# kkromberg/SpeechRecognition

Hardware: AMD Instinct MI355X
Metric: frames/sec scored+decoded (higher is better)
Workload: dtype f64

## Files before the change

### speechrecognition_amd/csrc/gmm_prefilter.hip

```cpp
#include <hip/hip_runtime.h>
#include <stdint.h>

#include <algorithm>
#include <cmath>
#include <vector>

#include "kernels.h"

#ifndef SR_P16_NB
#define SR_P16_NB 4
#endif

namespace srgpu {

typedef float v4f __attribute__((ext_vector_type(4)));
static constexpr int kPWaves = 4;
static constexpr int kGroupBlocks = 8;

typedef _Float16 f16x8 __attribute__((ext_vector_type(8)));

__device__ inline uint32_t pack_f16x2(_Float16 l, _Float16 h) {
  return (uint32_t)__builtin_bit_cast(uint16_t, l) | ((uint32_t)__builtin_bit_cast(uint16_t, h) << 16);
}

// ... 330 lines not shown
  if (e == hipSuccess) e = hipStreamSynchronize(stream);
  if (e == hipSuccess) e = hipMemcpy(h, d, sizeof(h), hipMemcpyDeviceToHost);
  (void)hipFree(d);
  if (e != hipSuccess) return e;
  *preserved = true;
  for (int i = 0; i < 64; i++) *preserved = *preserved && h[i] == 9.765625e-4f;
  return hipSuccess;
}

template <int KS>
__global__ void fp16_accumulation_probe_kernel(const _Float16* A, const _Float16* B, float* out) {
  constexpr int K = 32 * KS;
  const int lane = threadIdx.x, r = lane & 15, q = lane >> 4;
  v4f acc = {0.f, 0.f, 0.f, 0.f};
#pragma unroll
  for (int ks = 0; ks < KS; ks++) {
    f16x8 a, b;
#pragma unroll
    for (int j = 0; j < 8; j++) {
      const int k = 32 * ks + 8 * q + j;
      a[j] = A[r * K + k];
      b[j] = B[k * 16 + r];
    }
    acc = __builtin_amdgcn_mfma_f32_16x16x32_f16(a, b, acc, 0, 0, 0);
  }
#pragma unroll
  for (int i = 0; i < 4; i++) out[(4 * q + i) * 16 + r] = acc[i];
}

hipError_t probe_fp16_accumulation(hipStream_t stream, int ks32, bool* ok, double* worst_ratio) {
  if (ks32 != 3 && ks32 != 4) return hipErrorInvalidValue;
  const int kCases = 8;
  const int K = 32 * ks32;
  const double allowed = ks32 == 3 ? 87.0 : 132.0;
  std::vector<_Float16> hA((size_t)kCases * 16 * K), hB((size_t)kCases * K * 16);
  uint64_t rng = 0x9E3779B97F4A7C15ull;
  auto next = [&]() { rng ^= rng << 13; rng ^= rng >> 7; rng ^= rng << 17; return rng; };
  for (int t = 0; t < kCases; t++) {
    _Float16* A = hA.data() + (size_t)t * 16 * K;
    _Float16* B = hB.data() + (size_t)t * K * 16;
    for (int k = 0; k < K; k++)
      for (int c = 0; c < 16; c++) B[k * 16 + c] = (_Float16)1.0f;
    for (int r = 0; r < 16; r++)
      for (int k = 0; k < K; k++) {
        float a = 0.f;
        const int fam = (t * 16 + r) & 3;
        if (fam == 0) a = k == (r * 5) % K ? 4096.0f : 0.75f;
        else if (fam == 1) a = k >= K - 2 ? 0.f : ((k & 1) ? -1.f : 1.f) * (1024.0f + (float)(((k >> 1) * 7 + r) % 64) * ((k & 1) ? 0.5f : 0.53125f));
        else if (fam == 2) a = 1.0009765625f;
        else { const uint64_t u = next(); a = ((u & 1) ? -1.f : 1.f) * (1.0f + (float)((u >> 8) & 1023) / 1024.0f) * (float)(1u << ((u >> 20) % 12)); }
        A[r * K + k] = (_Float16)a;
      }
    for (int k = 0; k < K; k++)
      for (int c = 0; c < 16; c++) {
        const uint64_t u = next();
        float b = 1.0f + (float)((u >> 5) % 1024) / 1024.0f;
        if ((c & 3) == 0) b = 1.0f;
        if ((c & 3) == 1) b = 1.0009765625f;
        B[k * 16 + c] = (_Float16)b;
      }
    for (int c = 0; c < 16; c++)
      for (int r = 0; r < 16; r++)
        if (((t * 16 + r) & 3) == 0) B[((r * 5) % K) * 16 + c] = (_Float16)2048.0f;
  }
  _Float16 *dA = nullptr, *dB = nullptr;
  float* dO = nullptr;
  hipError_t e;
  if ((e = hipMalloc(reinterpret_cast<void**>(&dA), hA.size() * 2)) != hipSuccess) return e;
  if ((e = hipMalloc(reinterpret_cast<void**>(&dB), hB.size() * 2)) != hipSuccess) { (void)hipFree(dA); return e; }
  if ((e = hipMalloc(reinterpret_cast<void**>(&dO), (size_t)kCases * 256 * 4)) != hipSuccess) { (void)hipFree(dA); (void)hipFree(dB); return e; }
  std::vector<float> got((size_t)kCases * 256);
  e = hipMemcpy(dA, hA.data(), hA.size() * 2, hipMemcpyHostToDevice);
  if (e == hipSuccess) e = hipMemcpy(dB, hB.data(), hB.size() * 2, hipMemcpyHostToDevice);
  for (int t = 0; t < kCases && e == hipSuccess; t++) {
    if (ks32 == 3) hipLaunchKernelGGL(fp16_accumulation_probe_kernel<3>, dim3(1), dim3(64), 0, stream, dA + (size_t)t * 16 * K, dB + (size_t)t * K * 16, dO + (size_t)t * 256);
    else hipLaunchKernelGGL(fp16_accumulation_probe_kernel<4>, dim3(1), dim3(64), 0, stream, dA + (size_t)t * 16 * K, dB + (size_t)t * K * 16, dO + (size_t)t * 256);
    e = hipGetLastError();
  }
  if (e == hipSuccess) e = hipStreamSynchronize(stream);
  if (e == hipSuccess) e = hipMemcpy(got.data(), dO, got.size() * 4, hipMemcpyDeviceToHost);
  (void)hipFree(dA); (void)hipFree(dB); (void)hipFree(dO);
  if (e != hipSuccess) return e;
  double worst = 0.0;
  bool fine = true;
  for (int t = 0; t < kCases; t++)
    for (int r = 0; r < 16; r++)
      for (int c = 0; c < 16; c++) {
        double exact = 0.0, mag = 0.0;
        for (int k = 0; k < K; k++) {
          const double p = (double)(float)hA[((size_t)t * 16 + r) * K + k] * (double)(float)hB[((size_t)t * K + k) * 16 + c];
          exact += p;
          mag += p < 0 ? -p : p;
        }
        const double err = std::fabs((double)got[(size_t)t * 256 + r * 16 + c] - exact);
        const double ratio = err / (mag * 5.9604644775390625e-8);
        if (!(ratio <= allowed)) fine = false;
        if (ratio > worst || ratio != ratio) worst = ratio;
      }
  *ok = fine;
  if (worst_ratio) *worst_ratio = worst;
  return hipSuccess;
}

static GmmStationaryPlan stationary_plan(uint32_t n_groups, uint64_t n_frames) {
  GmmStationaryPlan p{};
  p.n_quads = (n_groups + kPWaves - 1) / kPWaves;
  const uint64_t steps = (n_frames + 16 * kSNB - 1) / (16 * kSNB);
  const uint64_t r_max = std::max<uint64_t>(1, std::min<uint64_t>(steps, (n_frames + kSRangeFrames - 1) / kSRangeFrames));
  uint64_t best_r = 1;
  double best = -1.0;
  for (uint64_t r = 1; r <= r_max; r++) {
    const uint64_t wgs = (uint64_t)p.n_quads * r;
    const double fill = (double)wgs / (double)((wgs + 511) / 512 * 512);
    if (fill > best * (1.0 + 1e-9)) { best = fill; best_r = r; }
  }
  const uint64_t range_steps = (steps + best_r - 1) / best_r;
  p.range_frames = (uint32_t)(range_steps * 16 * kSNB);
  p.n_ranges = (uint32_t)((steps + range_steps - 1) / range_steps);
  p.per_xcd = (uint32_t)(((uint64_t)p.n_quads * p.n_ranges + 7) / 8);
  return p;
}

int gmm_prefilter_route(int ks32, int route) { return (route == kPfStationary && ks32 >= 1 && ks32 <= 3) ? kPfStationary : kPfStaged; }
int gmm_prefilter_stationary_range_frames() { return kSRangeFrames; }
void gmm_prefilter_operand_sizes(int ks32, uint64_t n_frames, size_t* n_frag, size_t* n_norm) {
  const uint64_t blocks = (n_frames + 16 * kSNB - 1) / (16 * kSNB) * kSNB;
  *n_frag = (size_t)blocks * ks32 * 64;
  *n_norm = (size_t)blocks * 16;
}

template <int KS32>
static hipError_t launch_stationary(const GmmPrefilterArgs& a, hipStream_t stream) {
  if (!a.bfrag || !a.bnorm || a.n_groups == 0) return hipErrorInvalidValue;
  size_t n_frag, n_norm;
  gmm_prefilter_operand_sizes(KS32, a.n_frames, &n_frag, &n_norm);
  const uint64_t blocks = n_norm / 16;
  hipLaunchKernelGGL((gmm_prefilter_operands_kernel<KS32>), dim3((unsigned)((blocks + kPWaves - 1) / kPWaves)), dim3(kPWaves * 64), 0, stream,
                     a.feats, a.n_frames, a.dim, blocks, a.bfrag, a.bnorm);
  hipError_t e = hipGetLastError();
  if (e != hipSuccess) return e;
  const GmmStationaryPlan p = stationary_plan(a.n_groups, a.n_frames);
  hipLaunchKernelGGL((gmm_prefilter_stationary_kernel<KS32>), dim3(8 * p.per_xcd), dim3(kPWaves * 64), 0, stream, a, p);
  return hipGetLastError();
}

hipError_t launch_gmm_prefilter(const GmmPrefilterArgs& a, int ks32, int route, hipStream_t stream) {
  if (a.n_frames >= (1ull << 30)) return hipErrorInvalidValue;
  if (a.n_frames == 0) return hipSuccess;
  if (gmm_prefilter_route(ks32, route) == kPfStationary) {
    switch (ks32) {
      case 1: return launch_stationary<1>(a, stream);
      case 2: return launch_stationary<2>(a, stream);
      default: return launch_stationary<3>(a, stream);
    }
  }
  const dim3 grid(a.nx * a.ny), block(kPWaves * 64);
  switch (ks32) {
    case 1: hipLaunchKernelGGL((gmm_prefilter16_kernel<1, SR_P16_NB>), grid, block, 0, stream, a); break;
    case 2: hipLaunchKernelGGL((gmm_prefilter16_kernel<2, SR_P16_NB>), grid, block, 0, stream, a); break;
    case 3: hipLaunchKernelGGL((gmm_prefilter16_kernel<3, SR_P16_NB>), grid, block, 0, stream, a); break;
    case 4: hipLaunchKernelGGL((gmm_prefilter16_kernel<4, SR_P16_NB>), grid, block, 0, stream, a); break;
    default: return hipErrorInvalidValue;
  }
  return hipGetLastError();
}
int gmm_prefilter_frames_per_tile() { return kPWaves * SR_P16_NB * 16; }

#pragma clang fp contract(off)

#ifndef SR_R_THREADS
#define SR_R_THREADS 768
#endif
#ifndef SR_R_BATCH
#define SR_R_BATCH 4
#endif
static constexpr int kRThreads = SR_R_THREADS;
static constexpr int kRThreadsWide = 512;
static constexpr int kRWaves = kRThreads / 64;
static constexpr int kRBatch = SR_R_BATCH;
#ifndef SR_R_BATCH_WIDE
#define SR_R_BATCH_WIDE 8
#endif
static constexpr int kRBatchWide = SR_R_BATCH_WIDE;
static constexpr uint32_t kRingEntries = 128;
static constexpr uint32_t kRingLists = 2 * 8 * kRingEntries;
static constexpr uint32_t kRingWave = 4 * kRingLists;
struct __attribute__((aligned(16))) RingEntry { uint32_t lf, mask; double score; };
struct __attribute__((packed, aligned(4))) RowPiece { float v[4]; };

template <int DT, int NS, int SPW, int CH, int NT = kRThreads, int VS = 1, bool DEFER = false>
__global__ __launch_bounds__(NT) void gmm_refine_kernel(GmmRefineArgs a) {
  static_assert(DT > 0 && (DT & 1), "padded dimension: odd");
  static_assert(!DEFER || CH > 1, "deferred lists: states of several chunks");
  constexpr int kRThreads = NT, kRWaves = NT / 64;
  static_assert(CH == 1 || CH == 2 || CH == 4, "chunks per state (half)");
  static_assert(VS == 1 || (VS == 2 && CH == 4), "two halves only of four-chunk states");
  static_assert(SPW % (CH * VS) == 0 && (CH == 1 || SPW % 4 == 0), "a state's chunks live in one workgroup");
  extern __shared__ __attribute__((aligned(1024))) unsigned char panel_raw[];
  const uint32_t D = (uint32_t)DT, tid = threadIdx.x;
  const int lane = tid & 63, wave = tid >> 6;
  const uint32_t s0 = blockIdx.x * SPW;
  const uint32_t ns = (s0 + SPW <= a.n_pstates) ? SPW : a.n_pstates - s0;
  const uint32_t state_bytes = (2u * D + 2u) * NS * 8u;
  const uint64_t f_begin = (uint64_t)blockIdx.y * a.frames_per_split;
  const uint64_t f_end = (f_begin + a.frames_per_split < a.n_frames) ? f_begin + a.frames_per_split : a.n_frames;

  {
    const uint32_t chunks = (ns * state_bytes + 1023u) >> 10;
    const unsigned char* src = reinterpret_cast<const unsigned char*>(a.rows) + (uint64_t)s0 * state_bytes + lane * 16;
    for (uint32_t ch = wave; ch < chunks; ch += kRWaves)
      __builtin_amdgcn_global_load_lds((const __attribute__((address_space(1))) void*)(src + (uint64_t)ch * 1024u),
                                       (__attribute__((address_space(3))) void*)(panel_raw + ch * 1024u), 16, 0, 0);
  }
  uint32_t nd[SPW];
#pragma unroll
  for (int j = 0; j < SPW; j++) nd[j] = (uint32_t)j < ns ? a.n_dens_ps[s0 + j] : 0u;
  __builtin_amdgcn_s_waitcnt(0x0F70);
  __syncthreads();
  if (f_begin >= f_end) return;

  uint32_t n_eval = 0;
  double x[DT];
  const __amdgpu_buffer_rsrc_t featsT_rsrc = __builtin_amdgcn_make_buffer_rsrc(
      const_cast<float*>(a.featsT), 0, (int)0xFFFFFFFFu, 0x00020000);
  const uint32_t ld4 = (uint32_t)a.n_frames_ld * 4u;
  auto load_x = [&](uint64_t f) __attribute__((always_inline)) {
    const uint32_t voff = (uint32_t)f * 4u;
#pragma unroll
    for (int k = 0; k < DT; k++)
      x[k] = (double)__builtin_bit_cast(float, __builtin_amdgcn_raw_buffer_load_b32(featsT_rsrc, voff, (uint32_t)k * ld4, 0));
  };
  auto load_x_row = [&](uint64_t f) __attribute__((always_inline)) {
    const float* xr = a.feats + f * (uint64_t)DT;
#pragma unroll
    for (int q = 0; q < DT / 4; q++) {
      const RowPiece t = reinterpret_cast<const RowPiece*>(xr)[q];
#pragma unroll
      for (int i = 0; i < 4; i++) x[4 * q + i] = (double)t.v[i];
    }
#pragma unroll
    for (int k = DT - DT % 4; k < DT; k++) x[k] = (double)xr[k];
  };
  auto evaluate = [&](const unsigned char* col0) __attribute__((always_inline)) -> double {
    const volatile __attribute__((address_space(3))) double* col =
        (const volatile __attribute__((address_space(3))) double*)col0;
    double l0 = 0.0, l1 = 0.0, dist, score;
    {
      constexpr int RB = NT == kRThreadsWide ? kRBatchWide : kRBatch;
      constexpr int NB_ = (DT + 1 + RB - 1) / RB;
      double pm[2][RB], pv[2][RB];
#pragma unroll
      for (int i = 0; i < RB; i++)
        if (i <= DT) { pm[0][i] = col[(2 * i) * NS]; pv[0][i] = col[(2 * i + 1) * NS]; }
#pragma unroll
      for (int b = 0; b < NB_; b++) {
        const int cur = b & 1;
        __builtin_amdgcn_sched_barrier(0);
#pragma unroll
        for (int i = 0; i < RB; i++) {
          const int k = (b + 1) * RB + i;
          if (k <= DT) { pm[cur ^ 1][i] = col[(2 * k) * NS]; pv[cur ^ 1][i] = col[(2 * k + 1) * NS]; }
        }
        __builtin_amdgcn_sched_barrier(0);
#pragma unroll
        for (int i = 0; i < RB; i++) {
          const int k = b * RB + i;
          if (k < (int)(DT - (DT & 1))) {
            double u = x[k] - pm[cur][i];
            u = u * u;
            u = u * pv[cur][i];
            if (k & 1) l1 = l1 + u; else l0 = l0 + u;
          } else if (k == DT - 1) {
            dist = l0 + l1;
            const double t = x[k] - pm[cur][i];
            dist += t * t * pv[cur][i];
          } else if (k == DT) {
            if (!(DT & 1)) dist = l0 + l1;
            score = pm[cur][i] + dist / 2;
            score -= pv[cur][i];
          }
        }
        asm volatile("" : "+v"(l0), "+v"(l1));
      }
    }
    return score;
  };

  const double seed = 1e10;
  auto seeded_min = [&](double score) -> double {
    double r;
    asm("v_min_f64 %0, %1, %2" : "=v"(r) : "v"(score), "s"(seed));
    return r;
  };
  RingEntry* ring = reinterpret_cast<RingEntry*>(a.ring + ((uint64_t)(blockIdx.y * gridDim.x + blockIdx.x) * kRWaves + wave) * kRingWave);
  const bool counting = a.n_refined != nullptr;
  uint64_t cnt1 = 0, cnt2 = 0;
  const uint64_t wave_global = (uint64_t)(blockIdx.y * gridDim.x + blockIdx.x) * kRWaves + wave;
  RingEntry* seg = DEFER ? reinterpret_cast<RingEntry*>(a.defer) + wave_global * SPW * (uint64_t)a.defer_cap : nullptr;
  uint32_t dcnt[DEFER ? SPW : 1];
  if constexpr (DEFER) {
#pragma unroll
    for (int j = 0; j < SPW; j++) dcnt[j] = 0;
  }
  const uint64_t f_wave = f_begin + (uint64_t)wave * 64;
  auto frame_of = [&](uint32_t lf) -> uint64_t { return f_wave + (uint64_t)(lf >> 6) * kRThreads + (lf & 63u); };
  const uint32_t chunk_shift = CH == 1 ? (a.chunks == 1 ? 0u : a.chunks == 2 ? 1u : 2u) : CH == 2 ? 1u : VS == 2 ? 3u : 2u;

  const uint32_t n_it = (uint32_t)((f_end - f_begin + kRThreads - 1) / kRThreads);
  for (uint32_t it = 0; it < n_it; it++) {
    const uint64_t fr = f_wave + (uint64_t)it * kRThreads + lane;
    const bool valid = fr < f_end;
    const uint64_t f = valid ? fr : f_end - 1;
    const uint32_t lf = it * 64u + (uint32_t)lane;
    load_x(f);
    constexpr int RS = SPW / (CH * VS);
    double res[RS];
    if constexpr (CH == 1) {
#pragma unroll
      for (int h = 0; h < SPW / 4; h++) {
        const uint4 v = reinterpret_cast<const uint4*>(a.mask)[(uint64_t)((s0 >> 2) + h) * a.n_frames + f];
        const uint32_t mk[4] = {v.x, v.y, v.z, v.w};
#pragma unroll
        for (int jj = 0; jj < 4; jj++) {
          const int j = 4 * h + jj;
          const uint32_t n = nd[j];
          uint32_t mask = mk[jj];
          mask &= n >= 32 ? 0xFFFFFFFFu : ((1u << n) - 1u);
          res[j] = 1e10;
          if (n) {
            const double score = evaluate(panel_raw + (size_t)j * state_bytes + (uint32_t)__builtin_ctz(mask | 0x80000000u) * 8u);
            res[j] = mask != 0 ? seeded_min(score) : res[j];
            if (counting) n_eval += (uint32_t)__builtin_popcountll(__ballot(valid));
          }
          const bool more = valid && (mask & (mask - 1)) != 0;
          const uint64_t b = __ballot(more);
          if (b) {
            const uint32_t c1 = (uint32_t)(cnt1 >> (8 * j)) & 0xFFu;
            const uint32_t pos = c1 + __builtin_amdgcn_mbcnt_hi((uint32_t)(b >> 32), __builtin_amdgcn_mbcnt_lo((uint32_t)b, 0u));
            if (more) {
              ring[(uint32_t)j * kRingEntries + pos] = RingEntry{lf, mask & (mask - 1), res[j]};
            }
            cnt1 += (uint64_t)__builtin_popcountll(b) << (8 * j);
          }
        }
      }
      if (valid) {
        if (a.chunks == 1) {
          double* o = a.out + f * a.ld + s0;
          if (ns == SPW) {
#pragma unroll
            for (int j = 0; j < SPW; j += 2) *reinterpret_cast<double2*>(o + j) = make_double2(res[j], res[j + 1]);
          } else {
#pragma unroll
            for (int j = 0; j < SPW; j++)
              if ((uint32_t)j < ns) o[j] = res[j];
          }
        } else if (a.chunks == 2) {
          double* o = a.out + f * a.ld + s0 / 2;
#pragma unroll
          for (int j = 0; j < SPW; j += 2) {
            const double m = res[j + 1] < res[j] ? res[j + 1] : res[j];
            if ((uint32_t)j < ns) o[j / 2] = m;
          }
        } else {
          double* o = a.out + f * a.ld + s0 / 4;
#pragma unroll
          for (int j = 0; j < SPW; j += 4) {
            double m = res[j + 1] < res[j] ? res[j + 1] : res[j];
            m = res[j + 2] < m ? res[j + 2] : m;
            m = res[j + 3] < m ? res[j + 3] : m;
            if ((uint32_t)j < ns) o[j / 4] = m;
          }
        }
      }
    } else {
      auto append = [&](int j, bool more, uint32_t rest, double& best) __attribute__((always_inline)) {
        const uint64_t b = __ballot(more);
        if (b) {
          if constexpr (DEFER) {
            const uint32_t nb = (uint32_t)__builtin_popcountll(b);
            if (dcnt[DEFER ? j : 0] + nb <= a.defer_cap) {
              const uint32_t pos = dcnt[DEFER ? j : 0] + __builtin_amdgcn_mbcnt_hi((uint32_t)(b >> 32), __builtin_amdgcn_mbcnt_lo((uint32_t)b, 0u));
              if (more) seg[(uint64_t)j * a.defer_cap + pos] = RingEntry{(uint32_t)f, rest, best};
              dcnt[DEFER ? j : 0] += nb;
            } else {
              uint32_t mm = more ? rest : 0u;
              const unsigned char* panel = panel_raw + (size_t)j * state_bytes;
              do {
                const double score = evaluate(panel + (uint32_t)__builtin_ctz(mm | 0x80000000u) * 8u);
                if (counting) n_eval += (uint32_t)__builtin_popcountll(__ballot(mm != 0));
                if (mm != 0 && score < best) best = score;
                mm &= mm - 1;
              } while (__any(mm != 0));
            }
          } else {
          const uint32_t c1 = (uint32_t)(cnt1 >> (8 * j)) & 0xFFu;
          const uint32_t pos = c1 + __builtin_amdgcn_mbcnt_hi((uint32_t)(b >> 32), __builtin_amdgcn_mbcnt_lo((uint32_t)b, 0u));
          if (more) {
            ring[(uint32_t)j * kRingEntries + pos] = RingEntry{lf, rest, best};
          }
          cnt1 += (uint64_t)__builtin_popcountll(b) << (8 * j);
          }
        }
      };
      uint32_t mk[SPW];
#pragma unroll
      for (int h = 0; h < SPW / 4; h++) {
        const uint4 v = reinterpret_cast<const uint4*>(a.mask)[(uint64_t)((s0 >> 2) + h) * a.n_frames + f];
        mk[4 * h] = v.x; mk[4 * h + 1] = v.y; mk[4 * h + 2] = v.z; mk[4 * h + 3] = v.w;
      }
#pragma unroll
      for (int j = 0; j < SPW; j++) mk[j] &= nd[j] >= 32 ? 0xFFFFFFFFu : ((1u << nd[j]) - 1u);
      if constexpr (VS == 1) {
#pragma unroll
      for (int r = 0; r < RS; r++) {
        uint32_t msel = mk[r * CH], off = 0;
#pragma unroll
        for (int c = 1; c < CH; c++) {
          const bool empty = msel == 0;
          msel = empty ? mk[r * CH + c] : msel;
          off = empty ? (uint32_t)c * state_bytes : off;
        }
        res[r] = 1e10;
        if (nd[r * CH]) {
          const double score = evaluate(panel_raw + (size_t)(r * CH) * state_bytes + off + (uint32_t)__builtin_ctz(msel | 0x80000000u) * 8u);
          res[r] = msel != 0 ? seeded_min(score) : res[r];
          if (counting) n_eval += (uint32_t)__builtin_popcountll(__ballot(valid));
        }
#pragma unroll
        for (int c = 0; c < CH; c++) {
          const bool is_sel = off == (uint32_t)c * state_bytes;
          const uint32_t rest = is_sel ? msel & (msel - 1) : mk[r * CH + c];
          if (nd[r * CH + c]) append(r * CH + c, valid && rest != 0, rest, res[r]);
        }
      }
      } else {
#pragma unroll
      for (int r = 0; r < RS; r++) res[r] = 1e10;
#pragma unroll
      for (int rv = 0; rv < RS * VS; rv++) {
        uint32_t msel = mk[rv * CH], off = 0;
#pragma unroll
        for (int c = 1; c < CH; c++) {
          const bool empty = msel == 0;
          msel = empty ? mk[rv * CH + c] : msel;
          off = empty ? (uint32_t)c * state_bytes : off;
        }
        double resv = 1e10;
        if (nd[rv * CH]) {
          const double score = evaluate(panel_raw + (size_t)(rv * CH) * state_bytes + off + (uint32_t)__builtin_ctz(msel | 0x80000000u) * 8u);
          resv = msel != 0 ? seeded_min(score) : resv;
          if (counting) n_eval += (uint32_t)__builtin_popcountll(__ballot(valid));
        }
        if constexpr (VS == 1) res[rv] = resv;
        else res[rv / VS] = resv < res[rv / VS] ? resv : res[rv / VS];
#pragma unroll
        for (int c = 0; c < CH; c++) {
          const bool is_sel = off == (uint32_t)c * state_bytes;
          const uint32_t rest = is_sel ? msel & (msel - 1) : mk[rv * CH + c];
          if (nd[rv * CH + c]) append(rv * CH + c, valid && rest != 0, rest, resv);
        }
        if constexpr (DEFER && VS == 2) res[rv / VS] = resv < res[rv / VS] ? resv : res[rv / VS];
      }
      }
      if (valid) {
        double* o = a.out + f * a.ld + s0 / (CH * VS);
        if (ns == SPW && RS >= 2) {
#pragma unroll
          for (int r = 0; r + 1 < RS; r += 2) *reinterpret_cast<double2*>(o + r) = make_double2(res[r], res[r + 1]);
        } else {
#pragma unroll
          for (int r = 0; r < RS; r++)
            if ((uint32_t)(r * CH * VS) < ns) o[r] = res[r];
        }
      }
    }
    const bool last = it + 1 == n_it;
    if constexpr (!DEFER)
    for (;;) {
      uint32_t level, j, n;
      {
        const uint64_t full1 = cnt1 & 0x4040404040404040ull, full2 = cnt2 & 0x4040404040404040ull;
        const uint64_t pick2 = full2 ? full2 : (last && !full1 && !cnt1) ? cnt2 : 0;
        const uint64_t pick1 = full2 ? 0 : full1 ? full1 : last ? cnt1 : 0;
        const uint64_t pick = pick1 ? pick1 : pick2;
        if (!pick) break;
        level = pick1 ? 1u : 2u;
        j = (uint32_t)__builtin_ctzll(pick) >> 3;
        const uint32_t have_ = (uint32_t)((pick1 ? cnt1 : cnt2) >> (8u * j)) & 0xFFu;
        n = have_ < 64u ? have_ : 64u;
      }
      asm volatile("" : "+s"(level), "+s"(j), "+s"(n));
      const bool l1 = level == 1;
      const uint32_t have = (uint32_t)((l1 ? cnt1 : cnt2) >> (8u * j)) & 0xFFu;
      const uint32_t slot0 = ((level - 1u) * 8u + j) * kRingEntries;
      if (l1) cnt1 -= (uint64_t)n << (8u * j); else cnt2 -= (uint64_t)n << (8u * j);
      const bool live = (uint32_t)lane < n;
      asm volatile("" ::: "memory");
      __builtin_amdgcn_fence(__ATOMIC_RELEASE, "wavefront");
      __builtin_amdgcn_fence(__ATOMIC_ACQUIRE, "wavefront");
      asm volatile("" ::: "memory");
      const uint32_t at = slot0 + have - n + (live ? (uint32_t)lane : 0u);
      const RingEntry en = ring[at];
      const uint32_t lfb = en.lf;
      uint32_t m = live ? en.mask : 0u;
      double cur = en.score;
      const uint64_t fb = frame_of(lfb);
      load_x_row(fb);
      double* o = a.out + fb * a.ld + ((s0 + j) >> chunk_shift);
      if constexpr (CH == 1) {
        if (chunk_shift) cur = *o;
      }
      const double before = cur;
      const unsigned char* panel = panel_raw + (size_t)j * state_bytes;
      do {
        const double score = evaluate(panel + (uint32_t)__builtin_ctz(m | 0x80000000u) * 8u);
        if (counting) n_eval += (uint32_t)__builtin_popcountll(__ballot(m != 0));
        if (m != 0 && score < cur) cur = score;
        m &= m - 1;
      } while (!l1 && __any(m != 0));
      if (l1) {
        const uint64_t b = __ballot(m != 0);
        if (b) {
          const uint32_t c2 = (uint32_t)(cnt2 >> (8u * j)) & 0xFFu;
          const uint32_t pos = c2 + __builtin_amdgcn_mbcnt_hi((uint32_t)(b >> 32), __builtin_amdgcn_mbcnt_lo((uint32_t)b, 0u));
          if (m != 0) {
            ring[(8u + j) * kRingEntries + pos] = RingEntry{lfb, m, cur};
          }
          cnt2 += (uint64_t)__builtin_popcountll(b) << (8u * j);
        }
      }
      asm volatile("" ::: "memory");
      const bool lower = live && cur < before;
      if constexpr (CH == 1) {
        if (lower) *o = cur;
      } else {
        __builtin_amdgcn_fence(__ATOMIC_RELEASE, "wavefront");
        if (lower) (void)__builtin_amdgcn_global_atomic_fmin_f64((__attribute__((address_space(1))) double*)o, cur);
      }
    }
  }
  if constexpr (DEFER) {
#pragma unroll
    for (int j = 0; j < SPW; j++)
      if (lane == 0) a.defer_cnt[wave_global * SPW + j] = dcnt[j];
  }
  if (a.n_refined) {
    if (lane == 0) atomicAdd(a.n_refined, (unsigned long long)n_eval);
  }
}

template <int DT, int NS, int SPW, int CH, int NT, int VS>
__global__ __launch_bounds__(NT) void gmm_drain_kernel(GmmRefineArgs a) {
  constexpr int kRWaves = NT / 64;
  constexpr int RB = kRBatch;
  extern __shared__ __attribute__((aligned(1024))) unsigned char panel_raw[];
  const uint32_t tid = threadIdx.x;
  const int lane = tid & 63, wave = tid >> 6;
  const uint32_t s0 = blockIdx.x * SPW;
  const uint32_t ns = (s0 + SPW <= a.n_pstates) ? SPW : a.n_pstates - s0;
  const uint32_t state_bytes = (2u * DT + 2u) * NS * 8u;
  {
    const uint32_t chunks = (ns * state_bytes + 1023u) >> 10;
    const unsigned char* src = reinterpret_cast<const unsigned char*>(a.rows) + (uint64_t)s0 * state_bytes + lane * 16;
    for (uint32_t ch = wave; ch < chunks; ch += kRWaves)
      __builtin_amdgcn_global_load_lds((const __attribute__((address_space(1))) void*)(src + (uint64_t)ch * 1024u),
                                       (__attribute__((address_space(3))) void*)(panel_raw + ch * 1024u), 16, 0, 0);
  }
  const uint64_t wave_global = (uint64_t)(blockIdx.y * gridDim.x + blockIdx.x) * kRWaves + wave;
  const RingEntry* seg = reinterpret_cast<const RingEntry*>(a.defer) + wave_global * SPW * (uint64_t)a.defer_cap;
  RingEntry* ring = reinterpret_cast<RingEntry*>(a.ring + wave_global * kRingWave) + 8u * kRingEntries;
  uint32_t nj[SPW];
#pragma unroll
  for (int j = 0; j < SPW; j++) nj[j] = (uint32_t)j < ns ? (uint32_t)__builtin_amdgcn_readfirstlane((int)a.defer_cnt[wave_global * SPW + j]) : 0u;
  __builtin_amdgcn_s_waitcnt(0x0F70);
  __syncthreads();
  const bool counting = a.n_refined != nullptr;
  uint32_t n_eval = 0;
  constexpr uint32_t chunk_shift = CH == 2 ? 1u : VS == 2 ? 3u : 2u;
  uint64_t cnt2 = 0;

  float xf[DT];
  auto load_row = [&](uint64_t f) __attribute__((always_inline)) {
    const float* xr = a.feats + f * (uint64_t)DT;
#pragma unroll
    for (int q = 0; q < DT / 4; q++) {
      const RowPiece t = reinterpret_cast<const RowPiece*>(xr)[q];
#pragma unroll
      for (int i = 0; i < 4; i++) xf[4 * q + i] = t.v[i];
    }
#pragma unroll
    for (int k = DT - DT % 4; k < DT; k++) xf[k] = xr[k];
  };
  auto evaluate = [&](const unsigned char* col0) __attribute__((always_inline)) -> double {
    const volatile __attribute__((address_space(3))) double* col = (const volatile __attribute__((address_space(3))) double*)col0;
    double l0 = 0.0, l1 = 0.0, dist, score;
    constexpr int NB_ = (DT + 1 + RB - 1) / RB;
    double pm[2][RB], pv[2][RB];
#pragma unroll
    for (int i = 0; i < RB; i++)
      if (i <= DT) { pm[0][i] = col[(2 * i) * NS]; pv[0][i] = col[(2 * i + 1) * NS]; }
#pragma unroll
    for (int b = 0; b < NB_; b++) {
      const int cur = b & 1;
      __builtin_amdgcn_sched_barrier(0);
#pragma unroll
      for (int i = 0; i < RB; i++) {
        const int k = (b + 1) * RB + i;
        if (k <= DT) { pm[cur ^ 1][i] = col[(2 * k) * NS]; pv[cur ^ 1][i] = col[(2 * k + 1) * NS]; }
      }
      __builtin_amdgcn_sched_barrier(0);
#pragma unroll
      for (int i = 0; i < RB; i++) {
        const int k = b * RB + i;
        if (k < DT - 1) {
          double u = (double)xf[k < DT ? k : 0] - pm[cur][i];
          u = u * u;
          u = u * pv[cur][i];
          if (k & 1) l1 = l1 + u; else l0 = l0 + u;
        } else if (k == DT - 1) {
          dist = l0 + l1;
          const double t = (double)xf[k < DT ? k : 0] - pm[cur][i];
          dist += t * t * pv[cur][i];
        } else if (k == DT) {
          score = pm[cur][i] + dist / 2;
          score -= pv[cur][i];
        }
      }
      asm volatile("" : "+v"(l0), "+v"(l1));
    }
    return score;
  };
  auto batch = [&](const bool l1, const uint32_t j, const RingEntry en, const bool live) __attribute__((always_inline)) {
    uint32_t m = live ? en.mask : 0u;
    double cur = en.score;
    const uint64_t fb = en.lf;
    load_row(fb);
    double* o = a.out + fb * a.ld + ((s0 + j) >> chunk_shift);
    const double before = cur;
    const unsigned char* panel = panel_raw + (size_t)j * state_bytes;
    do {
      const double score = evaluate(panel + (uint32_t)__builtin_ctz(m | 0x80000000u) * 8u);
      if (counting) n_eval += (uint32_t)__builtin_popcountll(__ballot(m != 0));
      if (m != 0 && score < cur) cur = score;
      m &= m - 1;
    } while (!l1 && __any(m != 0));
    if (l1) {
      const uint64_t b = __ballot(m != 0);
      if (b) {
        const uint32_t c2 = (uint32_t)(cnt2 >> (8u * j)) & 0xFFu;
        const uint32_t pos = c2 + __builtin_amdgcn_mbcnt_hi((uint32_t)(b >> 32), __builtin_amdgcn_mbcnt_lo((uint32_t)b, 0u));
        if (m != 0) ring[j * kRingEntries + pos] = RingEntry{en.lf, m, cur};
        cnt2 += (uint64_t)__builtin_popcountll(b) << (8u * j);
      }
    }
    if (live && cur < before) (void)__builtin_amdgcn_global_atomic_fmin_f64((__attribute__((address_space(1))) double*)o, cur);
  };
  auto level2 = [&](const bool flush) __attribute__((always_inline)) {
    for (;;) {
      const uint64_t pick = (cnt2 & 0x4040404040404040ull) ? (cnt2 & 0x4040404040404040ull) : flush ? cnt2 : 0ull;
      if (!pick) break;
      uint32_t j = (uint32_t)__builtin_ctzll(pick) >> 3;
      asm volatile("" : "+s"(j));
      const uint32_t have = (uint32_t)(cnt2 >> (8u * j)) & 0xFFu, n = have < 64u ? have : 64u;
      cnt2 -= (uint64_t)n << (8u * j);
      const bool live = (uint32_t)lane < n;
      asm volatile("" ::: "memory");
      __builtin_amdgcn_fence(__ATOMIC_RELEASE, "wavefront");
      __builtin_amdgcn_fence(__ATOMIC_ACQUIRE, "wavefront");
      asm volatile("" ::: "memory");
      const RingEntry en = ring[j * kRingEntries + have - n + (live ? (uint32_t)lane : 0u)];
      batch(false, j, en, live);
    }
  };
#pragma unroll 1
  for (uint32_t j = 0; j < ns; j++) {
    uint32_t n_left = 0;
#pragma unroll
    for (int q = 0; q < SPW; q++) n_left = (uint32_t)q == j ? nj[q] : n_left;
    const RingEntry* sj = seg + (uint64_t)j * a.defer_cap;
    RingEntry nxt = n_left ? sj[(uint32_t)lane < n_left ? lane : 0] : RingEntry{0u, 0u, 0.0};
#pragma unroll 1
    for (uint32_t pos = 0; pos < n_left; pos += 64u) {
      const RingEntry en = nxt;
      const uint32_t n = n_left - pos < 64u ? n_left - pos : 64u;
      const uint32_t p2 = pos + 64u;
      if (p2 < n_left) nxt = sj[p2 + ((uint32_t)lane < n_left - p2 ? lane : 0)];
      batch(true, j, en, (uint32_t)lane < n);
      level2(false);
    }
  }
  level2(true);
  if (a.n_refined) {
    if (lane == 0) atomicAdd(a.n_refined, (unsigned long long)n_eval);
  }
}

__device__ inline uint32_t padded_source_dim(uint32_t k, uint32_t dim, uint32_t dp) {
  const uint32_t pairs = dim - (dim & 1u);
  return k < pairs ? k : (k == dp - 1u && (dim & 1u)) ? dim - 1u : dim;
}
__global__ void transpose_feats_kernel(const float* feats, uint64_t n_frames, uint32_t dim, uint32_t dp, uint64_t ldT, float* out, float* featsP) {
  __shared__ float tile[64][65];
  const uint64_t f0 = (uint64_t)blockIdx.x * 64;
  for (uint32_t d0 = 0; d0 < dp; d0 += 64) {
    for (uint32_t i = threadIdx.x; i < 64 * 64; i += blockDim.x) {
      const uint32_t fr = i / 64, d = i % 64;
      const uint32_t src = d0 + d < dp ? padded_source_dim(d0 + d, dim, dp) : dim;
      tile[fr][d] = (f0 + fr < n_frames && src < dim) ? feats[(f0 + fr) * dim + src] : 0.0f;
    }
    __syncthreads();
    for (uint32_t i = threadIdx.x; i < 64 * 64; i += blockDim.x) {
      const uint32_t d = i / 64, fr = i % 64;
      if (f0 + fr < n_frames && d0 + d < dp) out[(uint64_t)(d0 + d) * ldT + f0 + fr] = tile[fr][d];
    }
    if (featsP) {
      for (uint32_t i = threadIdx.x; i < 64 * 64; i += blockDim.x) {
        const uint32_t fr = i / 64, d = i % 64;
        if (f0 + fr < n_frames && d0 + d < dp) featsP[(f0 + fr) * dp + d0 + d] = tile[fr][d];
      }
    }
    __syncthreads();
  }
}

hipError_t launch_transpose_feats(const float* feats, uint64_t n_frames, uint32_t dim, uint32_t dp, uint64_t ldT, float* out, float* featsP,
                                  hipStream_t stream) {
  if (n_frames == 0) return hipSuccess;
  if (dp < dim || (dp != dim && !featsP)) return hipErrorInvalidValue;
  hipLaunchKernelGGL(transpose_feats_kernel, dim3((unsigned)((n_frames + 63) / 64)), dim3(256), 0, stream, feats, n_frames, dim, dp, ldT, out,
                     dp != dim ? featsP : nullptr);
  return hipGetLastError();
}

int gmm_refine_slots(uint32_t max_dens, uint32_t padded_dim) { return padded_dim > 39 ? 32 : max_dens <= 8 ? 8 : max_dens <= 16 ? 16 : 32; }

uint32_t gmm_refine_padded_dim(uint32_t dim) {
  static const uint32_t bounds[] = {9, 17, 25, 33, 39, 47, 55, 63};
  const uint32_t need = dim | 1u;
  for (uint32_t b : bounds)
    if (need <= b) return b;
  return 0;
}

static int refine_threads(uint32_t dp) { return dp <= 47 ? kRThreads : kRThreadsWide; }
static int refine_spw(const GmmRefineArgs& a) {
  return (size_t)(2 * a.dim + 2) * a.n_slots * 8 * 8 <= 160 * 1024 ? 8 : 4;
}
static void refine_grid(const GmmRefineArgs& a, int spw, uint32_t* n_sgroups, uint64_t* splits, uint64_t* frames_per_split) {
  const uint64_t nt = (uint64_t)refine_threads(a.dim);
  *n_sgroups = (a.n_pstates + spw - 1) / spw;
  uint64_t sp = std::max<uint64_t>(1, (512 + *n_sgroups - 1) / *n_sgroups);
  sp = std::min<uint64_t>(sp, (a.n_frames + nt - 1) / nt);
  sp = std::max<uint64_t>(sp, 1);
  *frames_per_split = (a.n_frames + sp - 1) / sp;
  *splits = *frames_per_split ? (a.n_frames + *frames_per_split - 1) / *frames_per_split : 1;
}
size_t gmm_refine_ring_words(const GmmRefineArgs& a) {
  uint32_t g; uint64_t sp, fps;
  refine_grid(a, refine_spw(a), &g, &sp, &fps);
  return (size_t)g * sp * kRWaves * kRingWave;
}

void gmm_refine_geometry(const GmmRefineArgs& a, uint32_t out[4]) {
  uint32_t g; uint64_t sp, fps;
  const int spw = refine_spw(a);
  refine_grid(a, spw, &g, &sp, &fps);
  out[0] = (uint32_t)refine_threads(a.dim); out[1] = (uint32_t)spw; out[2] = (uint32_t)fps; out[3] = a.chunks;
}

static uint32_t defer_cap_for(const GmmRefineArgs& a, int spw) {
  uint32_t g; uint64_t sp, fps;
  refine_grid(a, spw, &g, &sp, &fps);
  const uint64_t per_wave = ((fps + kRThreads - 1) / kRThreads) * 64;
  return (uint32_t)std::min<uint64_t>(((per_wave / 4 + 63) & ~(uint64_t)63) + 64, 1u << 30);
}
void gmm_refine_defer_layout(const GmmRefineArgs& a, size_t budget_bytes, uint32_t cap_limit, uint32_t* cap, size_t* n_entries,
                             size_t* n_counts) {
  *cap = 0; *n_entries = 0; *n_counts = 0;
  if (a.chunks < 2 || a.dim > 39 || a.n_slots != 32 || a.n_frames == 0) return;
  uint32_t g; uint64_t sp, fps;
  refine_grid(a, 8, &g, &sp, &fps);
  uint32_t c = defer_cap_for(a, 8);
  if (cap_limit) c = std::min(c, cap_limit);
  const size_t segs = (size_t)g * sp * kRWaves * 8;
  if (segs * c * 16 > budget_bytes) return;
  *cap = c; *n_entries = segs * c; *n_counts = segs;
}

template <int DT, int NS, int SPW, int CH, int NT, int VS = 1>
static hipError_t launch_refine_one(const GmmRefineArgs& a0, hipStream_t stream) {
  GmmRefineArgs a = a0;
  const size_t state_bytes = (size_t)(2 * DT + 2) * NS * 8;
  const size_t smem = (SPW * state_bytes + 1023) & ~(size_t)1023;
  uint32_t n_sgroups;
  uint64_t splits;
  refine_grid(a, SPW, &n_sgroups, &splits, &a.frames_per_split);
  const dim3 grid(n_sgroups, (unsigned)splits), block(NT);
  if constexpr (CH > 1 && NT == kRThreads && SPW == 8) {
    if (a.defer && a.defer_cnt && a.defer_cap) {
      auto k1 = gmm_refine_kernel<DT, NS, SPW, CH, NT, VS, true>;
      auto k2 = gmm_drain_kernel<DT, NS, SPW, CH, NT, VS>;
      hipError_t e = hipFuncSetAttribute((const void*)k1, hipFuncAttributeMaxDynamicSharedMemorySize, (int)smem);
      if (e == hipSuccess) e = hipFuncSetAttribute((const void*)k2, hipFuncAttributeMaxDynamicSharedMemorySize, (int)smem);
      if (e != hipSuccess) return e;
      hipLaunchKernelGGL(k1, grid, block, smem, stream, a);
      if ((e = hipGetLastError()) != hipSuccess) return e;
      hipLaunchKernelGGL(k2, grid, block, smem, stream, a);
      return hipGetLastError();
    }
  }
  a.defer = nullptr; a.defer_cnt = nullptr; a.defer_cap = 0;
  auto kernel = gmm_refine_kernel<DT, NS, SPW, CH, NT, VS>;
  hipError_t e = hipFuncSetAttribute((const void*)kernel, hipFuncAttributeMaxDynamicSharedMemorySize, (int)smem);
  if (e != hipSuccess) return e;
  hipLaunchKernelGGL(kernel, grid, block, smem, stream, a);
  return hipGetLastError();
}

template <int DT>
static hipError_t launch_refine_narrow(const GmmRefineArgs& a, hipStream_t stream) {
  switch (a.n_slots) {
    case 8: return launch_refine_one<DT, 8, 8, 1, kRThreads>(a, stream);
    case 16: return launch_refine_one<DT, 16, 8, 1, kRThreads>(a, stream);
    case 32:
      if (a.chunks == 2) return launch_refine_one<DT, 32, 8, 2, kRThreads>(a, stream);
      if (a.chunks == 4) return launch_refine_one<DT, 32, 8, 4, kRThreads>(a, stream);
      if (a.chunks == 8) return launch_refine_one<DT, 32, 8, 4, kRThreads, 2>(a, stream);
      return launch_refine_one<DT, 32, 8, 1, kRThreads>(a, stream);
    default: return hipErrorInvalidValue;
  }
}
template <int DT>
static hipError_t launch_refine_wide(const GmmRefineArgs& a, hipStream_t stream) {
  if (a.n_slots != 32) return hipErrorInvalidValue;
  if (a.chunks == 2) return launch_refine_one<DT, 32, 4, 2, kRThreadsWide>(a, stream);
  if (a.chunks == 4) return launch_refine_one<DT, 32, 4, 4, kRThreadsWide>(a, stream);
  return launch_refine_one<DT, 32, 4, 1, kRThreadsWide>(a, stream);
}

hipError_t launch_gmm_refine(const GmmRefineArgs& a, hipStream_t stream) {
  if (a.n_frames == 0) return hipSuccess;
  if (!a.ring || (uint64_t)a.dim * a.n_frames_ld * 4u >= (1ull << 32)) return hipErrorInvalidValue;
  if (a.chunks != 1 && (a.n_slots != 32 || (a.chunks != 2 && a.chunks != 4 && a.chunks != 8))) return hipErrorInvalidValue;
  if (a.chunks == 8 && a.dim > 39) return hipErrorInvalidValue;
  switch (a.dim) {
    case 9: return launch_refine_narrow<9>(a, stream);
    case 17: return launch_refine_narrow<17>(a, stream);
    case 25: return launch_refine_narrow<25>(a, stream);
    case 33: return launch_refine_narrow<33>(a, stream);
    case 39: return launch_refine_narrow<39>(a, stream);
    case 47:
      if (a.n_slots != 32) return hipErrorInvalidValue;
      return a.chunks == 2 ? launch_refine_one<47, 32, 4, 2, kRThreads>(a, stream) : a.chunks == 4 ? launch_refine_one<47, 32, 4, 4, kRThreads>(a, stream)
                           : launch_refine_one<47, 32, 4, 1, kRThreads>(a, stream);
    case 55: return launch_refine_wide<55>(a, stream);
    case 63: return launch_refine_wide<63>(a, stream);
    default: return hipErrorInvalidValue;
  }
}

}
```

### speechrecognition_amd/csrc/kernels.h

```cpp
#pragma once
#include <hip/hip_runtime.h>
#include <stdint.h>

#include <vector>

#include "bigram_route.h"

namespace srgpu {

struct GmmMfmaArgs {
  const float* feats;
  uint64_t n_frames;
  uint32_t dim;
  const double* apack;
  const uint32_t* blk_meta;
  const uint32_t* grp_state;
  const uint32_t* split_begin;
  double* out;
  uint32_t ld;
  uint32_t nx, ny;
};
int gmm_mfma_ksteps_for_dim(uint32_t dim);
int gmm_mfma_frames_per_tile(int ksteps);
hipError_t launch_gmm_mfma(const GmmMfmaArgs& a, int ksteps, bool sum, hipStream_t stream);

struct GmmExactArgs {
  const float* feats;
  uint64_t n_frames;
  uint32_t dim;
  uint32_t n_states;
  const uint32_t* dens_off;
  const double* means;
  const double* inv_vars;
  const double* norm;
  const double* logw;
  double* out;
  uint32_t ld;
  uint32_t states_per_split;
};
hipError_t launch_gmm_exact(const GmmExactArgs& a, bool sum, uint32_t n_splits, hipStream_t stream);
struct GmmExactList {
  const uint64_t* blk_frame0;
  const uint32_t* blk_frames;
  const uint32_t* blk_list;
  const uint32_t* list_off;
  const uint32_t* states;
  uint32_t blk_first;
  uint64_t frame_base;
};
hipError_t launch_gmm_exact_listed(const GmmExactArgs& a, bool sum, const GmmExactList& L, uint32_t n_blocks, hipStream_t stream);
int gmm_exact_frames_per_block();

struct GmmPrefilterArgs {
  const float* feats;
  uint64_t n_frames;
  uint32_t dim;
  const unsigned char* apack;
  const float* grp_lim;
  const uint32_t* split_begin;
  uint32_t* mask;
  uint32_t nx, ny;
  uint32_t chunks;
  uint32_t n_groups;
  uint4* bfrag;
  float2* bnorm;
};
enum { kPfStaged = 0, kPfStationary = 1 };
struct PfBound { float kappa, acc, abs, sub; };
constexpr float kPfRes16 = 4.8835e-4f;
inline constexpr PfBound pf_bound(int ks32) {
  return ks32 == 4 ? PfBound{1.05e-3f, 1.6e-5f, 7.0e-7f, 3.38e-7f} : PfBound{1.05e-3f, 1.1e-5f, 6.0e-7f, 2.92e-7f};
}
struct GmmRefineArgs {
  const float* feats;
  const float* featsT;
  uint64_t n_frames, n_frames_ld;
  uint32_t dim, n_pstates, chunks;
  const uint32_t* n_dens_ps;
  const double* rows;
  uint32_t n_slots;
  const uint32_t* mask;
  double* out; uint32_t ld;
  uint64_t frames_per_split;
  unsigned long long* n_refined;
  uint32_t* ring;
  void* defer;
  uint32_t* defer_cnt;
  uint32_t defer_cap;
};
void gmm_refine_defer_layout(const GmmRefineArgs& a, size_t budget_bytes, uint32_t cap_limit, uint32_t* cap, size_t* n_entries,
                             size_t* n_counts);
size_t gmm_refine_ring_words(const GmmRefineArgs& a);
void gmm_refine_geometry(const GmmRefineArgs& a, uint32_t out[4]);
hipError_t launch_gmm_prefilter(const GmmPrefilterArgs& a, int ks32, int route, hipStream_t stream);
int gmm_prefilter_route(int ks32, int route);
int gmm_prefilter_frames_per_tile();
int gmm_prefilter_stationary_range_frames();
void gmm_prefilter_operand_sizes(int ks32, uint64_t n_frames, size_t* n_frag, size_t* n_norm);
hipError_t probe_fp16_denormals(hipStream_t stream, bool* preserved);
hipError_t probe_fp16_accumulation(hipStream_t stream, int ks32, bool* ok, double* worst_ratio);
uint32_t gmm_refine_padded_dim(uint32_t dim);
int gmm_refine_slots(uint32_t max_dens, uint32_t padded_dim);
hipError_t launch_gmm_refine(const GmmRefineArgs& a, hipStream_t stream);
hipError_t launch_transpose_feats(const float* feats, uint64_t n_frames, uint32_t dim, uint32_t dp, uint64_t ldT, float* out, float* featsP,
                                  hipStream_t stream);

struct DecodeNet {
  uint32_t n_slots;
  uint32_t n_words;
  const uint32_t* slot_info;
  const uint32_t* slot_word;
  const uint32_t* word_end_slot;
  uint32_t silence_word;
  double tdp_loop, tdp_forward, tdp_skip;
  uint32_t silence_state;
};
static constexpr uint32_t kSlotPos0 = 1u << 16;
static constexpr uint32_t kSlotPos1 = 1u << 17;
static constexpr uint32_t kSlotEnd = 1u << 18;
static constexpr uint32_t kSlotSilState = 1u << 19;
static constexpr uint32_t kSlotSilWord = 1u << 20;
static constexpr uint32_t kSlotFirstSil = 1u << 21;
static constexpr uint32_t kSlotSingle = 1u << 22;
struct FastNet {
  uint32_t n_slots;
  const uint32_t* state;
  const uint32_t* pred;
  const uint32_t* orig;
  const uint32_t* chunk_type;
  const uint32_t* word;
  uint32_t init_slot;
  uint32_t init_is_end;
};
struct WordNet {
  const uint32_t* info;
  const uint2* states;
  const uint32_t* order;
  uint32_t nw, nt;
  uint32_t plain_len;
  uint32_t has_general;
  uint32_t init_is_end;
};
struct DecodeArgs {
  DecodeNet net;
  FastNet fast;
  WordNet words;
  const double* scores;
  uint32_t ld;
  const uint64_t* frame_off;
  uint64_t frame_base;
  uint32_t utt_first, n_utts;
  const uint32_t* utt_order;
  double am_threshold, word_penalty;
  double* tb_score;
  uint16_t* tb_word;
  uint16_t* tb_bkp;
  uint32_t* out_words;
  uint32_t* out_count;
  uint32_t* out_flags;
  uint32_t only_flagged;
  uint32_t exact_negative;
};
enum class DecodeFirst { kNone, kWords, kSlots };
struct DecodeRoute {
  DecodeFirst first;
  bool big;
};
DecodeRoute decode_route(const DecodeArgs& a, bool general, bool slots);
hipError_t launch_decode(DecodeArgs a, const DecodeRoute& r, unsigned char* big_ws, hipStream_t stream);
uint32_t decode_max_slots();
uint32_t decode_big_max_slots();
size_t decode_big_workspace(uint32_t n_slots);
uint32_t decode_words_max_words();
hipError_t launch_decode_fast(const DecodeArgs& a, hipStream_t stream);
bool decode_words_applies(const DecodeArgs& a);
hipError_t launch_decode_words(const DecodeArgs& a, hipStream_t stream);
DecodeNet build_decode_net(uint32_t n_words, const uint32_t* word_off, const uint16_t* automaton, uint32_t silence_word,
                           uint32_t silence_state, const double tdp[3], std::vector<uint32_t>& slot_info,
                           std::vector<uint32_t>& slot_word, std::vector<uint32_t>& word_end_slot);
FastNet build_fast_net(const std::vector<uint32_t>& slot_info, const std::vector<uint32_t>& slot_word, const uint32_t* word_off,
                       std::vector<uint32_t>& state, std::vector<uint32_t>& pred, std::vector<uint32_t>& orig,
                       std::vector<uint32_t>& chunk_type, std::vector<uint32_t>& word);
WordNet build_word_net(uint32_t n_words, const uint32_t* word_off, const uint16_t* automaton, uint32_t silence_word,
                       uint32_t silence_state, std::vector<uint32_t>& info, std::vector<uint2>& states, std::vector<uint32_t>& order);
struct StreamState {
  double m_we;
  uint32_t e_first[4];
  uint32_t flags;
  uint32_t count;
  uint32_t pad[2];
};
struct StreamJob {
  uint32_t slot;
  uint32_t t0, k;
  uint32_t pad;
  uint64_t row0;
};
struct StreamArgs {
  DecodeNet net;
  double am_threshold, word_penalty;
  const double* scores;
  uint32_t ld;
  const StreamJob* jobs;
  unsigned char* ws;
  size_t ws_stride;
  StreamState* state;
  double* tb_score;
  uint16_t* tb_word;
  uint16_t* tb_bkp;
  uint64_t tb_stride;
  uint32_t* words;
  uint64_t words_stride;
};
hipError_t launch_decode_stream(const StreamArgs& a, uint32_t n_jobs, hipStream_t stream);
static constexpr uint32_t kStableCorrupt = 1u;
struct StableJob {
  uint32_t slot;
  uint32_t t;
  uint32_t fresh;
  uint32_t pad;
  uint64_t word_off;
};
struct StableResult {
  uint32_t commit;
  uint32_t silence;
  uint32_t count;
  uint32_t flags;
};
struct StableArgs {
  DecodeNet net;
  const StableJob* jobs;
  const unsigned char* ws;
  size_t ws_stride;
  const uint16_t* tb_word;
  const uint16_t* tb_bkp;
  uint64_t tb_stride;
  uint32_t* commit;
  uint32_t* words;
  uint64_t words_stride;
  StableResult* out_res;
  uint32_t* out_words;
};
hipError_t launch_stream_commit(const StableArgs& a, uint32_t n_jobs, hipStream_t stream);
struct CommitPointsArgs {
  const uint64_t* node_off;
  const uint32_t* parent;
  const uint64_t* set_off;
  const uint32_t* set;
  const uint32_t* floor;
  uint32_t* out;
};
hipError_t launch_commit_points(const CommitPointsArgs& a, uint32_t n_sets, hipStream_t stream);
hipError_t launch_traceback(const uint64_t* frame_off, uint32_t n_utts, const uint16_t* tb_word, const uint16_t* tb_bkp,
                            uint32_t silence_word, uint32_t n_words, uint32_t* out_words, uint32_t* out_count,
                            uint32_t* out_flags, hipStream_t stream);

constexpr uint32_t kGatherNone = 0xFFFFFFFFu;
constexpr int kGatherMaxArrays = 3;
struct GatherHeader {
  uint64_t n_words;
  uint32_t first_flagged;
  uint32_t first_over;
  uint32_t over_count;
  uint32_t reserved[3];
};
static_assert(sizeof(GatherHeader) == 32, "word_off follows the header, 8-byte aligned");
struct GatherArgs {
  const uint32_t* count;
  const uint32_t* flags;
  const uint64_t* frame_off;
  uint32_t n_utts, extra_slots, flag_mask;
  const uint32_t* src[kGatherMaxArrays];
  uint64_t* dev_off;
  unsigned char* block;
};
size_t gather_block_bytes(uint32_t n_utts, uint64_t n_slots, int n_arrays);
hipError_t launch_gather_words(const GatherArgs& a, int n_arrays, hipStream_t stream);

struct AlignArgs {
  const double* scores;
  uint32_t ld;
  const uint64_t* frame_off;
  uint64_t frame_base;
  uint32_t utt_first, n_utts;
  const uint32_t* utt_order;
  const uint16_t* automata;
  const uint64_t* aut_off;
  double tdp_loop, tdp_forward, tdp_skip;
  uint32_t silence_state;
  double pruning_threshold;
  uint8_t* backptr;
  const uint64_t* bp_off;
  uint32_t max_positions;
  uint16_t* out_states;
  double* out_cost;
};
hipError_t launch_align_full(const AlignArgs& a, hipStream_t stream);
hipError_t launch_align_pruned(const AlignArgs& a, hipStream_t stream);
uint32_t align_max_positions();
constexpr size_t kAlignLdsLimit = 160 * 1024;
constexpr size_t align_full_lds_bytes(uint32_t max_positions) { return (size_t)max_positions * (2 * 8 + 2) + 16; }
constexpr size_t align_pruned_lds_bytes(uint32_t max_positions) { return (size_t)max_positions * (2 * 8 + 2 + 2) + 4 * 8 + 16; }
constexpr uint32_t kAlignMaxPositions = 8192;
constexpr uint32_t kAlignPrunedMaxPositions = 8189;
static_assert(align_full_lds_bytes(kAlignMaxPositions) <= kAlignLdsLimit, "align_full_kernel at the position limit");
static_assert(align_pruned_lds_bytes(kAlignPrunedMaxPositions) <= kAlignLdsLimit &&
              align_pruned_lds_bytes(kAlignPrunedMaxPositions + 1) > kAlignLdsLimit, "align_pruned_kernel at the position limit");

struct FbArgs {
  const double* scores;
  uint32_t ld;
  uint64_t frame_base;
  const uint64_t* frame_off;
  uint32_t utt_first, n_utts;
  const uint16_t* automata;
  const uint64_t* aut_off;
  double tdp_loop, tdp_forward, tdp_skip;
  uint32_t silence_state;
  uint32_t max_positions;
  double* trellis;
  const uint64_t* trellis_off;
  double* out_cost;
};
hipError_t launch_fb_forward(const FbArgs& a, hipStream_t stream);
hipError_t launch_fb_backward(const FbArgs& a, hipStream_t stream);

struct ItemArgs {
  const uint64_t* frame_off;
  uint32_t utt_first, n_utts;
  uint64_t group_f0;
  const double* trellis;
  const uint64_t* trellis_off;
  const uint64_t* chain_off;
  uint32_t n_cols, n_mix;
  uint32_t row_stride;
  uint32_t serial_limit;
  const uint32_t* mix_off;
  const uint16_t* mix;
  const uint32_t* slot_beg;
  const uint16_t* slot_pos16;
  const uint32_t* slot_pos32;
  const double* gate;
  bool by_frame;
  double floor;
  uint32_t* group_cnt;
  const uint32_t* group_scan;
  uint32_t* item_base;
  uint32_t* item_off;
  uint32_t* item_frame; uint16_t* item_mix; double* item_w;
};
size_t items_scan_temp_bytes(uint64_t n_frames);
hipError_t launch_items(const ItemArgs& a, int sign, uint64_t n_frames, void* scan_temp, size_t scan_temp_bytes, uint32_t* scan_out,
                        hipStream_t stream);
hipError_t launch_items_top(const uint32_t* item_off, const uint16_t* item_mix, const double* item_w, uint64_t n_frames,
                            uint32_t max_items, uint16_t* out_count, uint16_t* out_state, double* out_weight, hipStream_t stream);

struct NetFbArgs {
  DecodeNet net;
  const double* scores;
  uint32_t ld;
  uint64_t frame_base;
  const uint64_t* frame_off;
  uint32_t utt_first, n_utts;
  double scale, word_penalty;
  uint64_t group_f0;
  double* trellis;
  double* out_cost;
  double* post;
  double* ends;
};
size_t netfb_max_slots();
hipError_t launch_netfb_forward(const NetFbArgs& a, hipStream_t stream);
hipError_t launch_netfb_backward(const NetFbArgs& a, hipStream_t stream);
hipError_t launch_netfb_words(const NetFbArgs& a, uint64_t n_frames, hipStream_t stream);
hipError_t launch_netfb_top(const NetFbArgs& a, uint64_t n_frames, uint32_t max_items, double floor, uint16_t* out_count,
                            uint32_t* out_word, double* out_weight, hipStream_t stream);
hipError_t launch_netfb_conf(const NetFbArgs& a, const uint16_t* tb_word, const uint16_t* tb_bkp, const uint32_t* out_count,
                             double* out_conf, uint32_t* out_first, uint32_t* out_last, hipStream_t stream);

hipError_t launch_netocc_backward(const NetFbArgs& a, hipStream_t stream);
struct ChainArgs {
  const double* scores;
  uint32_t ld;
  uint64_t frame_base;
  const uint64_t* frame_off;
  uint32_t utt_first, n_utts;
  double scale, word_penalty;
  double tdp_loop, tdp_forward, tdp_skip;
// ... 450 lines not shown
```

Baseline: 13.96 million.

## Distribute refine frame chunks to waves via per-block atomic tickets

In the non-deferred refine path, waves no longer take a fixed strided set of frame chunks. Each wave instead draws 64-frame chunk indices dynamically from a per-block atomic ticket counter kept after the ring buffer, which is zeroed with a memset before launch. This is meant to balance uneven per-wave refinement work, since waves can finish at different times because of the ring drains. It also hoists the mask loads ahead of load_x and prefetches the next ticket. The cost is one extra memset, one atomic per chunk, and a changed mapping from local frame index to frame.

```diff
diff --git a/speechrecognition_amd/csrc/gmm_prefilter.hip b/speechrecognition_amd/csrc/gmm_prefilter.hip
--- a/speechrecognition_amd/csrc/gmm_prefilter.hip
+++ b/speechrecognition_amd/csrc/gmm_prefilter.hip
@@ -656,23 +656,36 @@
 #pragma unroll
     for (int j = 0; j < SPW; j++) dcnt[j] = 0;
   }
+  constexpr bool DYN = !DEFER;
   const uint64_t f_wave = f_begin + (uint64_t)wave * 64;
-  auto frame_of = [&](uint32_t lf) -> uint64_t { return f_wave + (uint64_t)(lf >> 6) * kRThreads + (lf & 63u); };
+  auto frame_of = [&](uint32_t lf) -> uint64_t { return DYN ? f_begin + lf : f_wave + (uint64_t)(lf >> 6) * kRThreads + (lf & 63u); };
   const uint32_t chunk_shift = CH == 1 ? (a.chunks == 1 ? 0u : a.chunks == 2 ? 1u : 2u) : CH == 2 ? 1u : VS == 2 ? 3u : 2u;
 
-  const uint32_t n_it = (uint32_t)((f_end - f_begin + kRThreads - 1) / kRThreads);
-  for (uint32_t it = 0; it < n_it; it++) {
-    const uint64_t fr = f_wave + (uint64_t)it * kRThreads + lane;
+  const uint32_t n_loop = (uint32_t)((f_end - f_begin + (DYN ? 64 : kRThreads) - 1) / (DYN ? 64 : kRThreads));
+  uint32_t* ticket = a.tickets + (blockIdx.y * gridDim.x + blockIdx.x);
+  auto draw = [&]() -> uint32_t {
+    return lane == 0 ? __hip_atomic_fetch_add(ticket, 1u, __ATOMIC_RELAXED, __HIP_MEMORY_SCOPE_AGENT) : 0u;
+  };
+  uint32_t tk = 0, it = 0;
+  if constexpr (DYN) { tk = draw(); it = (uint32_t)__builtin_amdgcn_readfirstlane(tk); }
+  while (it < n_loop) {
+    const uint64_t fr = DYN ? f_begin + (uint64_t)it * 64 + lane : f_wave + (uint64_t)it * kRThreads + lane;
     const bool valid = fr < f_end;
     const uint64_t f = valid ? fr : f_end - 1;
     const uint32_t lf = it * 64u + (uint32_t)lane;
+    uint4 mq[CH == 1 ? SPW / 4 : 1];
+    if constexpr (CH == 1) {
+#pragma unroll
+      for (int h = 0; h < SPW / 4; h++) mq[h] = reinterpret_cast<const uint4*>(a.mask)[(uint64_t)((s0 >> 2) + h) * a.n_frames + f];
+    }
     load_x(f);
+    if constexpr (DYN) tk = draw();
     constexpr int RS = SPW / (CH * VS);
     double res[RS];
     if constexpr (CH == 1) {
 #pragma unroll
       for (int h = 0; h < SPW / 4; h++) {
-        const uint4 v = reinterpret_cast<const uint4*>(a.mask)[(uint64_t)((s0 >> 2) + h) * a.n_frames + f];
+        const uint4 v = mq[h];
         const uint32_t mk[4] = {v.x, v.y, v.z, v.w};
 #pragma unroll
         for (int jj = 0; jj < 4; jj++) {
@@ -829,7 +842,8 @@
         }
       }
     }
-    const bool last = it + 1 == n_it;
+    const uint32_t it_next = DYN ? (uint32_t)__builtin_amdgcn_readfirstlane(tk) : it + 1;
+    const bool last = it_next >= n_loop;
     if constexpr (!DEFER)
     for (;;) {
       uint32_t level, j, n;
@@ -893,6 +907,7 @@
         if (lower) (void)__builtin_amdgcn_global_atomic_fmin_f64((__attribute__((address_space(1))) double*)o, cur);
       }
     }
+    it = it_next;
   }
   if constexpr (DEFER) {
 #pragma unroll
@@ -1113,7 +1128,7 @@
 size_t gmm_refine_ring_words(const GmmRefineArgs& a) {
   uint32_t g; uint64_t sp, fps;
   refine_grid(a, refine_spw(a), &g, &sp, &fps);
-  return (size_t)g * sp * kRWaves * kRingWave;
+  return (size_t)g * sp * kRWaves * kRingWave + (size_t)g * sp;
 }
 
 void gmm_refine_geometry(const GmmRefineArgs& a, uint32_t out[4]) {
@@ -1151,6 +1166,8 @@
   uint64_t splits;
   refine_grid(a, SPW, &n_sgroups, &splits, &a.frames_per_split);
   const dim3 grid(n_sgroups, (unsigned)splits), block(NT);
+  a.tickets = a.ring + (size_t)n_sgroups * splits * kRWaves * kRingWave;
+  if (hipError_t e = hipMemsetAsync(a.tickets, 0, (size_t)n_sgroups * splits * sizeof(uint32_t), stream); e != hipSuccess) return e;
   if constexpr (CH > 1 && NT == kRThreads && SPW == 8) {
     if (a.defer && a.defer_cnt && a.defer_cap) {
       auto k1 = gmm_refine_kernel<DT, NS, SPW, CH, NT, VS, true>;
diff --git a/speechrecognition_amd/csrc/kernels.h b/speechrecognition_amd/csrc/kernels.h
--- a/speechrecognition_amd/csrc/kernels.h
+++ b/speechrecognition_amd/csrc/kernels.h
@@ -84,6 +84,7 @@
   uint64_t frames_per_split;
   unsigned long long* n_refined;
   uint32_t* ring;
+  uint32_t* tickets;
   void* defer;
   uint32_t* defer_cnt;
   uint32_t defer_cap;
```

Measured after the change: 14.60 million (median of 6 runs). 4.5% higher.
